# RS2002/PianoBart

Measured on AMD Instinct MI355X. Metric: Octuple tokens/sec/GPU (seq=1024, 12L/768d) pretrain step; %MFMA peak, higher is better.
Workload: dtype bf16

## Files before the change

### pianobart_amd/csrc/pb_fa_tiles.h

```cpp
#pragma once
#include "pb_common.h"
#include "pb_api_internal.h"

namespace {


constexpr int HD = 64, FT = 256;
constexpr float LOG2E = 1.4426950408889634f;
typedef __attribute__((ext_vector_type(4))) short s16x4;
typedef __attribute__((ext_vector_type(8))) short s16x8;

struct Fa64Args {
    const bf16_t *q, *k, *v, *o, *dout;
    bf16_t *out, *dq, *dk, *dv;
    float* lse; const float* delta; const float* key_mask; const int* kmax;
    int B, H, Sq, Sk;
    long q_sb, q_ss, k_sb, k_ss, v_sb, v_ss, o_sb, o_ss, dq_sb, dq_ss, dk_sb, dk_ss, dv_sb, dv_ss;
    float scale; int causal;
    float* cs_q; float* cs_kv;
    const bf16_t* zeros;
    const int *vl_q_off, *vl_k_off, *vl_q_len, *vl_k_len;
    const int* bh_order;
};

__device__ __forceinline__ void varlen_localize(Fa64Args& p, int b) {
    if (!p.vl_q_off) return;
    const long qo = p.vl_q_off[b], ko = p.vl_k_off[b];
    p.Sq = p.vl_q_len[b]; p.Sk = p.vl_k_len[b];
    p.q += qo * p.q_ss - b * p.q_sb; p.k += ko * p.k_ss - b * p.k_sb; p.v += ko * p.v_ss - b * p.v_sb;
    if (p.o) p.o += qo * p.o_ss - b * p.o_sb;
    if (p.out) p.out += qo * p.o_ss - b * p.o_sb;
    if (p.dout) p.dout += qo * p.o_ss - b * p.o_sb;
    if (p.dq) p.dq += qo * p.dq_ss - b * p.dq_sb;
    if (p.dk) p.dk += ko * p.dk_ss - b * p.dk_sb;
    if (p.dv) p.dv += ko * p.dv_ss - b * p.dv_sb;
}

#define MFMA16(a, b, c) __builtin_amdgcn_mfma_f32_16x16x32_bf16((a), (b), (c), 0, 0, 0)

__device__ __forceinline__ int fsw(int row) { return (((row >> 1) & 3) << 1) | ((row >> 3) & 1); }

__device__ __forceinline__ void glds16(const bf16_t* g, char* lds_wave_base) {
    __builtin_amdgcn_global_load_lds((const __attribute__((address_space(1))) void*)g,
                                     (__attribute__((address_space(3))) void*)lds_wave_base, 16, 0, 0);
}
struct StageOff { unsigned off[2]; unsigned chunk[2]; };
__device__ __forceinline__ StageOff stage_off(long ld, int wave, int lane) {
    StageOff o;
#pragma unroll
    for (int n = 0; n < 2; ++n) {
        const int row = (wave * 2 + n) * 8 + (lane >> 3);
        o.chunk[n] = (unsigned)((lane & 7) ^ fsw(row));
        o.off[n] = (unsigned)(row * ld + (o.chunk[n] << 3));
    }
    return o;
}
__device__ __forceinline__ void stage64(const bf16_t* __restrict__ base, long ld, int r0, int nrows, char* lds, int wave, int lane, const StageOff& so,
                                        int cmax = 8, const bf16_t* zeros = nullptr) {
    if (r0 + 64 <= nrows) {
        const bf16_t* tb = base + (long)r0 * ld;
#pragma unroll
        for (int n = 0; n < 2; ++n) glds16((cmax == 8 || (int)so.chunk[n] < cmax) ? tb + so.off[n] : zeros, lds + (wave * 2 + n) * 1024);
    } else {
#pragma unroll
        for (int n = 0; n < 2; ++n) {
            const int inst = wave * 2 + n;
            const int row = inst * 8 + (lane >> 3);
            const int chunk = (lane & 7) ^ fsw(row);
            const int gr = min(r0 + row, nrows - 1);
            glds16((cmax == 8 || chunk < cmax) ? base + (long)gr * ld + chunk * 8 : zeros, lds + inst * 1024);
        }
    }
}
__device__ __forceinline__ bf16x8 frag_row(const char* lds, int row, int ks, int g) {
    return *reinterpret_cast<const bf16x8*>(lds + row * 128 + (((ks * 4 + g) ^ fsw(row)) << 4));
}
__device__ __forceinline__ bf16x8 frag_tr(const char* lds, int c0, int s, int lane) {
    const int lr = lane & 15, g = lane >> 4, qq = lr >> 2, pp = lr & 3;
    const int chunk = (c0 >> 3) + (pp >> 1);
    const int r0 = 32 * s + 4 * g + qq, r1 = r0 + 16;
    const int o0 = r0 * 128 + ((chunk ^ fsw(r0)) << 4) + ((pp & 1) << 3);
    const int o1 = r1 * 128 + ((chunk ^ fsw(r1)) << 4) + ((pp & 1) << 3);
    const s16x4 lo = __builtin_amdgcn_ds_read_tr16_b64_v4i16((__attribute__((address_space(3))) s16x4*)(lds + o0));
    const s16x4 hi = __builtin_amdgcn_ds_read_tr16_b64_v4i16((__attribute__((address_space(3))) s16x4*)(lds + o1));
    const s16x8 v = {lo[0], lo[1], lo[2], lo[3], hi[0], hi[1], hi[2], hi[3]};
    return __builtin_bit_cast(bf16x8, v);
}
__device__ __forceinline__ bf16x8 pack_pair(const f32x4& lo, const f32x4& hi) {
    bf16x8 r = {(bf16_t)lo[0], (bf16_t)lo[1], (bf16_t)lo[2], (bf16_t)lo[3], (bf16_t)hi[0], (bf16_t)hi[1], (bf16_t)hi[2], (bf16_t)hi[3]};
    return r;
}
__device__ __forceinline__ bf16x8 frag_global(const bf16_t* __restrict__ g, long ld, int row, int nvalid, int col) {
    bf16x8 z = {};
    if (row < nvalid) z = *reinterpret_cast<const bf16x8*>(g + (long)row * ld + col);
    return z;
}
__device__ __forceinline__ float grp_max(float v) {
    auto a = __builtin_amdgcn_permlane16_swap(__float_as_uint(v), __float_as_uint(v), false, false);
    v = fmaxf(__uint_as_float(a[0]), __uint_as_float(a[1]));
    auto b = __builtin_amdgcn_permlane32_swap(__float_as_uint(v), __float_as_uint(v), false, false);
    return fmaxf(__uint_as_float(b[0]), __uint_as_float(b[1]));
}
__device__ __forceinline__ float grp_sum(float v) {
    auto a = __builtin_amdgcn_permlane16_swap(__float_as_uint(v), __float_as_uint(v), false, false);
    v = __uint_as_float(a[0]) + __uint_as_float(a[1]);
    auto b = __builtin_amdgcn_permlane32_swap(__float_as_uint(v), __float_as_uint(v), false, false);
    return __uint_as_float(b[0]) + __uint_as_float(b[1]);
}
template <bool V> struct BoolTag { static constexpr bool value = V; };

constexpr int STG = 2 * 8192 + 512;

__device__ __forceinline__ void block_map(int nrb, int H, int B, int& rb, int& h, int& b, const int* order = nullptr) {
    const int L = blockIdx.x, BH = H * B;
    int bh;
    if ((BH & 7) == 0) { const int x = L & 7, slot = L >> 3, j = slot / nrb; bh = j * 8 + x; rb = (slot - j * nrb + j) % nrb; }
    else { bh = L / nrb; rb = (L - bh * nrb + bh) % nrb; }
    if (order) bh = order[bh];
    h = bh % H; b = bh / H;
}

template <int OFF>
__device__ __forceinline__ void ds_tr(s16x4& d, unsigned addr) {
    asm volatile("ds_read_b64_tr_b16 %0, %1 offset:%2" : "=v"(d) : "v"(addr), "i"(OFF));
}
__device__ __forceinline__ unsigned tr_lane_off64(int c0, int lane) {
    const int lr = lane & 15, g = lane >> 4, qq = lr >> 2, pp = lr & 3;
    const int r0 = 4 * g + qq, chunk = (c0 >> 3) + (pp >> 1);
    return (unsigned)(r0 * 128 + ((chunk ^ fsw(r0)) << 4) + ((pp & 1) << 3));
}
__device__ __forceinline__ void ds_tr_block(s16x4 (&d)[2][2], unsigned addr) {
    ds_tr<0>(d[0][0], addr); ds_tr<2048>(d[0][1], addr); ds_tr<4096>(d[1][0], addr); ds_tr<6144>(d[1][1], addr);
}
__device__ __forceinline__ bf16x8 tr_join(s16x4 lo, s16x4 hi) {
    const s16x8 v = {lo[0], lo[1], lo[2], lo[3], hi[0], hi[1], hi[2], hi[3]};
    return __builtin_bit_cast(bf16x8, v);
}
#define TRW4(X) "+v"(X[0][0]), "+v"(X[0][1]), "+v"(X[1][0]), "+v"(X[1][1])
__device__ __forceinline__ void tr_wait4(s16x4 (&t)[4][2][2]) {
    asm volatile("s_waitcnt lgkmcnt(0)" : TRW4(t[0]), TRW4(t[1]), TRW4(t[2]), TRW4(t[3]));
}
__device__ __forceinline__ void tr_wait8(s16x4 (&t)[4][2][2], s16x4 (&u)[4][2][2]) {
    asm volatile("s_waitcnt lgkmcnt(0)" : TRW4(t[0]), TRW4(t[1]), TRW4(t[2]), TRW4(t[3]), TRW4(u[0]), TRW4(u[1]), TRW4(u[2]), TRW4(u[3]));
}
#undef TRW4
__device__ __forceinline__ unsigned lds_u32(const void* p) { return (unsigned)(uintptr_t)(__attribute__((address_space(3))) const char*)p; }

template <int N> __device__ __forceinline__ void wait_vm() { asm volatile("s_waitcnt vmcnt(%0)" :: "i"(N) : "memory"); }

template <int NB> struct FaCfg {
    static constexpr int NS = NB == 1 ? 3 : 2;
    static constexpr int STB = 2 * NB * 8192;
    static constexpr int PCS = 4 * NB;
    static constexpr int KT = NB == 1 ? 2 : 1;
};

__device__ __forceinline__ bf16x8 scale_frag(bf16x8 v, float c) {
    bf16x8 r;
#pragma unroll
    for (int e = 0; e < 8; ++e) r[e] = (bf16_t)((float)v[e] * c);
    return r;
}

}
```

### pianobart_amd/csrc/pb_flash64.hip

```cpp
#include "pb_common.h"
#include "pb_fa_tiles.h"

namespace {


constexpr float LAZY_THR = 8.0f;
template <int HD>
__global__ __launch_bounds__(FT) void fa64_fwd_kernel(const Fa64Args pin) {
    constexpr int NB = (HD + 63) / 64, KS = HD / 32, DT = HD / 16, HDT = HD;
    using C = FaCfg<NB>;
    extern __shared__ __attribute__((aligned(16))) char smem[];
    const int t = threadIdx.x, lane = t & 63, lr = lane & 15, g = lane >> 4;
    const int wave = __builtin_amdgcn_readfirstlane(t >> 6);
    int rb, h, b;
    block_map((pin.Sq + 127) / 128, pin.H, pin.B, rb, h, b, pin.bh_order);
    if (pin.causal) rb = (pin.Sq + 127) / 128 - 1 - rb;
    const int q0 = rb * 128;
    Fa64Args p = pin;
    varlen_localize(p, b);
    const int lse_ld = pin.Sq;
    if (q0 >= p.Sq) return;
    const bf16_t* Q = p.q + b * p.q_sb + h * HDT;
    const bf16_t* K = p.k + b * p.k_sb + h * HDT;
    const bf16_t* V = p.v + b * p.v_sb + h * HDT;
    const float c = p.scale * LOG2E;
    const int kvis_end = p.kmax ? min(p.Sk, p.kmax[b]) : p.Sk;
    const int kend = p.causal ? min(kvis_end, q0 + 128) : kvis_end;
    const int nt = (kend + 63) / 64;
    float* ldsBias = reinterpret_cast<float*>(smem + C::NS * C::STB);
    unsigned* ldsFlag = reinterpret_cast<unsigned*>(ldsBias + ((p.Sk + 63) / 64) * 64);
    for (int tile = wave; tile < nt; tile += 4) {
        const int key = tile * 64 + lane;
        const bool vis = key < (pin.vl_q_off ? kvis_end : p.Sk) && (!p.key_mask || p.key_mask[(long)b * p.Sk + key] != 0.f);
        ldsBias[key] = vis ? 0.f : -INFINITY;
        const bool allvis = __builtin_amdgcn_ballot_w64(vis) == ~0ull;
        if (lane == 0) ldsFlag[tile] = allvis ? 0u : 1u;
    }
    int myq[2];
    bf16x8 qf[2][KS];
#pragma unroll
    for (int qt = 0; qt < 2; ++qt) {
        myq[qt] = q0 + wave * 32 + qt * 16 + lr;
#pragma unroll
        for (int ks = 0; ks < KS; ++ks) qf[qt][ks] = scale_frag(frag_global(Q, p.q_ss, myq[qt], p.Sq, ks * 32 + g * 8), c);
    }
#pragma unroll
    for (int ks = 0; ks < KS; ++ks) asm volatile("" : "+v"(qf[0][ks]), "+v"(qf[1][ks]));
    f32x4 oacc[2][DT];
#pragma unroll
    for (int qt = 0; qt < 2; ++qt)
#pragma unroll
        for (int i = 0; i < DT; ++i) oacc[qt][i] = f32x4{0.f, 0.f, 0.f, 0.f};
    float m[2] = {-INFINITY, -INFINITY};
    f32x4 cinit[2] = {f32x4{0.f, 0.f, 0.f, 0.f}, f32x4{0.f, 0.f, 0.f, 0.f}};
    f32x4 lacc[2] = {f32x4{0.f, 0.f, 0.f, 0.f}, f32x4{0.f, 0.f, 0.f, 0.f}};
    const bf16_t one = (bf16_t)1.0f;
    const bf16x8 ones = {one, one, one, one, one, one, one, one};
    unsigned voff[4];
#pragma unroll
    for (int dt = 0; dt < 4; ++dt) voff[dt] = lds_u32(smem) + NB * 8192 + tr_lane_off64(dt * 16, lane);
    const StageOff so_k = stage_off(p.k_ss, wave, lane), so_v = stage_off(p.v_ss, wave, lane);
    auto stage = [&](int it, int sidx) {
        char* st = smem + sidx * C::STB;
#pragma unroll
        for (int nb = 0; nb < NB; ++nb) {
            stage64(K + nb * 64, p.k_ss, it * 64, p.Sk, st + nb * 8192, wave, lane, so_k, min(8, (HD - nb * 64) / 8), p.zeros);
            stage64(V + nb * 64, p.v_ss, it * 64, p.Sk, st + (NB + nb) * 8192, wave, lane, so_v, min(8, (HD - nb * 64) / 8), p.zeros);
        }
    };
    if (nt > 0) stage(0, 0);
    if (C::NS == 3 && nt > 1) { stage(1, 1); wait_vm<C::PCS>(); } else { wait_vm<0>(); }
    __builtin_amdgcn_s_waitcnt(0xc07f);
    __builtin_amdgcn_s_barrier();
    int sidx = 0;
    for (int it = 0; it < nt; ++it) {
        const char* st = smem + sidx * C::STB;
        const int nidx = sidx == 0 ? C::NS - 1 : sidx - 1;
        if (it + C::NS - 1 < nt) stage(it + C::NS - 1, nidx);
        const float* ldsB = ldsBias + it * 64;
        const int k0 = it * 64;
        const bool diag = p.causal && (k0 + 63 > q0 + wave * 32);
        const bool masked = diag || __builtin_amdgcn_readfirstlane(ldsFlag[it]) != 0u;
        f32x4 s[2][4];
#pragma unroll
        for (int kt = 0; kt < 4; ++kt) {
#pragma unroll
            for (int qt = 0; qt < 2; ++qt) s[qt][kt] = cinit[qt];
#pragma unroll
            for (int nb = 0; nb < NB; ++nb) {
#pragma unroll
                for (int k2 = 0; k2 < 2; ++k2)
                    if (2 * nb + k2 < KS) {
                        const bf16x8 kk = frag_row(st + nb * 8192, kt * 16 + lr, k2, g);
#pragma unroll
                        for (int qt = 0; qt < 2; ++qt) s[qt][kt] = MFMA16(kk, qf[qt][2 * nb + k2], s[qt][kt]);
                    }
            }
        }
        s16x4 tv[4][2][2];
#pragma unroll
        for (int dt = 0; dt < 4; ++dt) if (dt < DT) ds_tr_block(tv[dt], voff[dt] + (unsigned)(sidx * C::STB));
        bf16x8 pf[2][2];
        auto finish_row = [&](int qt) {
            pf[qt][0] = pack_pair(s[qt][0], s[qt][1]);
            pf[qt][1] = pack_pair(s[qt][2], s[qt][3]);
            lacc[qt] = MFMA16(ones, pf[qt][1], MFMA16(ones, pf[qt][0], lacc[qt]));
        };
        float resc[2] = {1.f, 1.f};
        auto exact_tile = [&](auto tag) {
            constexpr bool MASKED = decltype(tag)::value;
            asm volatile("; exact softmax path" ::: "memory");
#pragma unroll
            for (int qt = 0; qt < 2; ++qt) {
                const float mold = m[qt] == -INFINITY ? 0.f : m[qt];
                float mx = -INFINITY;
#pragma unroll
                for (int kt = 0; kt < 4; ++kt) {
                    f32x4 bias = {0.f, 0.f, 0.f, 0.f};
                    if constexpr (MASKED) bias = *reinterpret_cast<const f32x4*>(ldsB + kt * 16 + g * 4);
#pragma unroll
                    for (int r = 0; r < 4; ++r) {
                        float x = s[qt][kt][r] + mold;
                        if constexpr (MASKED) {
                            x += bias[r];
                            if (diag && (k0 + kt * 16 + g * 4 + r) > myq[qt]) x = -INFINITY;
                        }
                        s[qt][kt][r] = x;
                        mx = fmaxf(mx, x);
                    }
                }
                mx = grp_max(mx);
                const float mnew = fmaxf(m[qt], mx);
                const float muse = mnew == -INFINITY ? 0.f : mnew;
                const float alpha = __builtin_amdgcn_exp2f(m[qt] - muse);
#pragma unroll
                for (int kt = 0; kt < 4; ++kt)
#pragma unroll
                    for (int r = 0; r < 4; ++r) s[qt][kt][r] = __builtin_amdgcn_exp2f(s[qt][kt][r] - muse);
                lacc[qt] *= alpha;
                m[qt] = mnew;
                cinit[qt] = f32x4{-muse, -muse, -muse, -muse};
                resc[qt] = alpha;
                finish_row(qt);
            }
        };
        bool exact = masked;
        if (masked) {
            exact_tile(BoolTag<true>{});
        } else {
            float t0 = m[0] == -INFINITY ? INFINITY : -INFINITY, t1 = m[1] == -INFINITY ? INFINITY : -INFINITY;
#pragma unroll
            for (int kt = 0; kt < 4; ++kt)
#pragma unroll
                for (int r = 0; r < 4; ++r) { t0 = fmaxf(t0, s[0][kt][r]); t1 = fmaxf(t1, s[1][kt][r]); }
            if (__builtin_amdgcn_ballot_w64(fmaxf(t0, t1) > LAZY_THR) == 0ull) {
#pragma unroll
                for (int qt = 0; qt < 2; ++qt) {
#pragma unroll
                    for (int kt = 0; kt < 4; ++kt)
#pragma unroll
                        for (int r = 0; r < 4; ++r) s[qt][kt][r] = __builtin_amdgcn_exp2f(s[qt][kt][r]);
                    finish_row(qt);
                }
            } else {
                exact = true;
                exact_tile(BoolTag<false>{});
            }
        }
        if (exact) {
#pragma unroll
            for (int qt = 0; qt < 2; ++qt)
#pragma unroll
                for (int i = 0; i < DT; ++i) oacc[qt][i] *= resc[qt];
        }
#pragma unroll
        for (int nb = 0; nb < NB; ++nb) {
            if (nb > 0) {
#pragma unroll
                for (int dt = 0; dt < 4; ++dt) if (nb * 4 + dt < DT) ds_tr_block(tv[dt], voff[dt] + (unsigned)(sidx * C::STB + nb * 8192));
            }
            tr_wait4(tv);
#pragma unroll
            for (int dt = 0; dt < 4; ++dt) if (nb * 4 + dt < DT) {
                const bf16x8 v0 = tr_join(tv[dt][0][0], tv[dt][0][1]), v1 = tr_join(tv[dt][1][0], tv[dt][1][1]);
#pragma unroll
                for (int qt = 0; qt < 2; ++qt) oacc[qt][nb * 4 + dt] = MFMA16(v1, pf[qt][1], MFMA16(v0, pf[qt][0], oacc[qt][nb * 4 + dt]));
            }
        }
        if (C::NS == 3 && it + 2 < nt) { wait_vm<C::PCS>(); } else { wait_vm<0>(); }
        __builtin_amdgcn_s_barrier();
        sidx = sidx == C::NS - 1 ? 0 : sidx + 1;
    }
    if constexpr (HD == 64) {
        typedef __attribute__((ext_vector_type(2))) unsigned u32x2;
        typedef __attribute__((ext_vector_type(4))) unsigned u32x4;
        const unsigned obase = lds_u32(smem) + (unsigned)(wave * 4096);
#pragma unroll
        for (int qt = 0; qt < 2; ++qt) {
            const float lq = lacc[qt][0];
            const float inv = lq > 0.f ? 1.0f / lq : 0.f;
#pragma unroll
            for (int dt = 0; dt < DT; ++dt) {
                const bf16x4 r = {(bf16_t)(oacc[qt][dt][0] * inv), (bf16_t)(oacc[qt][dt][1] * inv), (bf16_t)(oacc[qt][dt][2] * inv), (bf16_t)(oacc[qt][dt][3] * inv)};
                *reinterpret_cast<__attribute__((address_space(3))) u32x2*>(obase + (unsigned)(qt * 2048 + lr * 128 + ((((dt * 2 + (g >> 1)) ^ (lr & 7)) << 4) | ((g & 1) << 3)))) =
                    __builtin_bit_cast(u32x2, r);
            }
            if (myq[qt] < p.Sq && g == 0) p.lse[((long)b * p.H + h) * lse_ld + myq[qt]] = lq > 0.f ? (m[qt] + log2f(lq)) / LOG2E : INFINITY;
        }
        const int orow = lane >> 3, ochunk = lane & 7;
#pragma unroll
        for (int qt = 0; qt < 2; ++qt)
#pragma unroll
            for (int hh = 0; hh < 2; ++hh) {
                const int r = hh * 8 + orow, q = q0 + wave * 32 + qt * 16 + r;
                const u32x4 v = *reinterpret_cast<const __attribute__((address_space(3))) u32x4*>(obase + (unsigned)(qt * 2048 + r * 128 + ((ochunk ^ (r & 7)) << 4)));
                if (q < p.Sq) *reinterpret_cast<u32x4*>(p.out + b * p.o_sb + (long)q * p.o_ss + h * HDT + ochunk * 8) = v;
            }
    } else {
#pragma unroll
    for (int qt = 0; qt < 2; ++qt) {
        if (myq[qt] < p.Sq) {
            const float lq = lacc[qt][0];
            const float inv = lq > 0.f ? 1.0f / lq : 0.f;
            bf16_t* O = p.out + b * p.o_sb + (long)myq[qt] * p.o_ss + h * HDT;
#pragma unroll
            for (int dt = 0; dt < DT; ++dt) {
                bf16x4 r = {(bf16_t)(oacc[qt][dt][0] * inv), (bf16_t)(oacc[qt][dt][1] * inv), (bf16_t)(oacc[qt][dt][2] * inv), (bf16_t)(oacc[qt][dt][3] * inv)};
                *reinterpret_cast<bf16x4*>(O + dt * 16 + g * 4) = r;
            }
            if (g == 0) p.lse[((long)b * p.H + h) * lse_ld + myq[qt]] = lq > 0.f ? (m[qt] + log2f(lq)) / LOG2E : INFINITY;
        }
    }
    }
}

template <int HD>
__global__ __launch_bounds__(FT) void fa64_bwd_dkv_kernel(const Fa64Args pin) {
    constexpr int NB = (HD + 63) / 64, KS = HD / 32, DT = HD / 16, HDT = HD;
    using C = FaCfg<NB>;
    constexpr int KT = C::KT, BK_ = 64 * KT;
    extern __shared__ __attribute__((aligned(16))) char smem[];
    const int t = threadIdx.x, lane = t & 63, lr = lane & 15, g = lane >> 4;
    const int wave = __builtin_amdgcn_readfirstlane(t >> 6);
    int rb, h, b;
    block_map((pin.Sk + BK_ - 1) / BK_, pin.H, pin.B, rb, h, b, pin.bh_order);
    const int k0 = rb * BK_;
    Fa64Args p = pin;
    varlen_localize(p, b);
    const int lse_ld = pin.Sq;
    if (k0 >= p.Sk) {
        if (p.cs_kv && t < 2 * HDT) {
            const int nkb0 = (pin.Sk + BK_ - 1) / BK_, dm = p.H * HDT;
            float* row = p.cs_kv + (long)(b * nkb0 + rb) * 2 * dm + h * HDT;
            row[t < HDT ? t : dm + t - HDT] = 0.f;
        }
        return;
    }
    const bf16_t* Q = p.q + b * p.q_sb + h * HDT;
    const bf16_t* K = p.k + b * p.k_sb + h * HDT;
    const bf16_t* V = p.v + b * p.v_sb + h * HDT;
    const bf16_t* DO = p.dout + b * p.o_sb + h * HDT;
    const float c = p.scale * LOG2E;
    const int it0 = p.causal ? k0 / 64 : 0;
    const int nt = (p.kmax && k0 >= p.kmax[b]) ? 0 : (p.Sq + 63) / 64;
    const int sqp = ((p.Sq + 63) / 64) * 64;
    float* ldsNL = reinterpret_cast<float*>(smem + C::NS * C::STB);
    float* ldsND = ldsNL + sqp;
    {
        const long li0 = ((long)b * p.H + h) * lse_ld;
        for (int qb = it0 * 64; qb < nt * 64; qb += 4 * FT) {
            float tl[4], td[4];
#pragma unroll
            for (int i = 0; i < 4; ++i) {
                const int q = qb + t + i * FT;
                tl[i] = q < p.Sq ? p.lse[li0 + q] : INFINITY;
                td[i] = q < p.Sq ? p.delta[li0 + q] : 0.f;
            }
#pragma unroll
            for (int i = 0; i < 4; ++i) {
                const int q = qb + t + i * FT;
                if (q < nt * 64) { ldsNL[q] = tl[i] == INFINITY ? -INFINITY : -tl[i] * LOG2E; ldsND[q] = -td[i]; }
            }
        }
    }
    int mykey[KT];
    bf16x8 kf[KT][KS], vf[KT][KS];
#pragma unroll
    for (int kt = 0; kt < KT; ++kt) {
        mykey[kt] = k0 + wave * (16 * KT) + kt * 16 + lr;
#pragma unroll
        for (int ks = 0; ks < KS; ++ks) {
            kf[kt][ks] = scale_frag(frag_global(K, p.k_ss, mykey[kt], p.Sk, ks * 32 + g * 8), c);
            vf[kt][ks] = frag_global(V, p.v_ss, mykey[kt], p.Sk, ks * 32 + g * 8);
        }
    }
#pragma unroll
    for (int kt = 0; kt < KT; ++kt)
#pragma unroll
        for (int ks = 0; ks < KS; ++ks) asm volatile("" : "+v"(kf[kt][ks]), "+v"(vf[kt][ks]));
    f32x4 dk[KT][DT], dv[KT][DT];
#pragma unroll
    for (int kt = 0; kt < KT; ++kt)
#pragma unroll
        for (int i = 0; i < DT; ++i) { dk[kt][i] = f32x4{0.f, 0.f, 0.f, 0.f}; dv[kt][i] = f32x4{0.f, 0.f, 0.f, 0.f}; }
    unsigned qoff[4], ooff[4];
#pragma unroll
    for (int dt = 0; dt < 4; ++dt) { qoff[dt] = lds_u32(smem) + tr_lane_off64(dt * 16, lane); ooff[dt] = qoff[dt] + NB * 8192; }
    const StageOff so_q = stage_off(p.q_ss, wave, lane), so_o = stage_off(p.o_ss, wave, lane);
    auto stage = [&](int it, int sidx) {
        char* st = smem + sidx * C::STB;
#pragma unroll
        for (int nb = 0; nb < NB; ++nb) {
            stage64(Q + nb * 64, p.q_ss, it * 64, p.Sq, st + nb * 8192, wave, lane, so_q, min(8, (HD - nb * 64) / 8), p.zeros);
            stage64(DO + nb * 64, p.o_ss, it * 64, p.Sq, st + (NB + nb) * 8192, wave, lane, so_o, min(8, (HD - nb * 64) / 8), p.zeros);
        }
    };
    if (it0 < nt) stage(it0, 0);
    if (C::NS == 3 && it0 + 1 < nt) { stage(it0 + 1, 1); wait_vm<C::PCS>(); } else { wait_vm<0>(); }
    __builtin_amdgcn_s_waitcnt(0xc07f);
    __builtin_amdgcn_s_barrier();
    int sidx = 0;
    for (int it = it0; it < nt; ++it) {
        const char* st = smem + sidx * C::STB;
        const int nidx = sidx == 0 ? C::NS - 1 : sidx - 1;
        if (it + C::NS - 1 < nt) stage(it + C::NS - 1, nidx);
        const int q0 = it * 64;
        const bool diag = p.causal && (k0 + wave * (16 * KT) + 16 * KT - 1 > q0);
        bf16x8 pf[KT][2], df[KT][2];
#pragma unroll
        for (int half = 0; half < 2; ++half) {
            f32x4 sv[KT][2], dp[KT][2];
#pragma unroll
            for (int qq = 0; qq < 2; ++qq) {
                const int qt = half * 2 + qq;
                const f32x4 nl = *reinterpret_cast<const f32x4*>(ldsNL + q0 + qt * 16 + g * 4);
                const f32x4 nd = *reinterpret_cast<const f32x4*>(ldsND + q0 + qt * 16 + g * 4);
#pragma unroll
                for (int kt = 0; kt < KT; ++kt) { sv[kt][qq] = nl; dp[kt][qq] = nd; }
#pragma unroll
                for (int nb = 0; nb < NB; ++nb) {
                    const char* ldsQ = st + nb * 8192; const char* ldsO = st + (NB + nb) * 8192;
#pragma unroll
                    for (int k2 = 0; k2 < 2; ++k2)
                        if (2 * nb + k2 < KS) {
                            const bf16x8 qa = frag_row(ldsQ, qt * 16 + lr, k2, g), oa = frag_row(ldsO, qt * 16 + lr, k2, g);
#pragma unroll
                            for (int kt = 0; kt < KT; ++kt) {
                                sv[kt][qq] = MFMA16(qa, kf[kt][2 * nb + k2], sv[kt][qq]);
                                dp[kt][qq] = MFMA16(oa, vf[kt][2 * nb + k2], dp[kt][qq]);
                            }
                        }
                }
            }
            if (diag) {
#pragma unroll
                for (int kt = 0; kt < KT; ++kt)
#pragma unroll
                    for (int qq = 0; qq < 2; ++qq)
#pragma unroll
                        for (int r = 0; r < 4; ++r) {
                            const int q = q0 + (half * 2 + qq) * 16 + g * 4 + r;
                            const float pr = mykey[kt] <= q ? __builtin_amdgcn_exp2f(sv[kt][qq][r]) : 0.f;
                            sv[kt][qq][r] = pr; dp[kt][qq][r] *= pr;
                        }
            } else {
#pragma unroll
                for (int kt = 0; kt < KT; ++kt)
#pragma unroll
                    for (int qq = 0; qq < 2; ++qq)
#pragma unroll
                        for (int r = 0; r < 4; ++r) {
                            const float pr = __builtin_amdgcn_exp2f(sv[kt][qq][r]);
                            sv[kt][qq][r] = pr; dp[kt][qq][r] *= pr;
                        }
            }
#pragma unroll
            for (int kt = 0; kt < KT; ++kt) { pf[kt][half] = pack_pair(sv[kt][0], sv[kt][1]); df[kt][half] = pack_pair(dp[kt][0], dp[kt][1]); }
        }
#pragma unroll
        for (int nb = 0; nb < NB; ++nb)
#pragma unroll
        for (int si = 0; si < 2; ++si) {
            s16x4 to[4][2], tq[4][2];
#pragma unroll
            for (int dt = 0; dt < 4; ++dt) if (nb * 4 + dt < DT) {
                const unsigned ao = ooff[dt] + (unsigned)(sidx * C::STB + nb * 8192), aq = qoff[dt] + (unsigned)(sidx * C::STB + nb * 8192);
                if (si == 0) { ds_tr<0>(to[dt][0], ao); ds_tr<2048>(to[dt][1], ao); ds_tr<0>(tq[dt][0], aq); ds_tr<2048>(tq[dt][1], aq); }
                else { ds_tr<4096>(to[dt][0], ao); ds_tr<6144>(to[dt][1], ao); ds_tr<4096>(tq[dt][0], aq); ds_tr<6144>(tq[dt][1], aq); }
            }
            asm volatile("s_waitcnt lgkmcnt(0)" : "+v"(to[0][0]), "+v"(to[0][1]), "+v"(to[1][0]), "+v"(to[1][1]), "+v"(to[2][0]), "+v"(to[2][1]), "+v"(to[3][0]), "+v"(to[3][1]),
                                                  "+v"(tq[0][0]), "+v"(tq[0][1]), "+v"(tq[1][0]), "+v"(tq[1][1]), "+v"(tq[2][0]), "+v"(tq[2][1]), "+v"(tq[3][0]), "+v"(tq[3][1]));
#pragma unroll
            for (int dt = 0; dt < 4; ++dt) if (nb * 4 + dt < DT) {
                const bf16x8 ot = tr_join(to[dt][0], to[dt][1]), qtf = tr_join(tq[dt][0], tq[dt][1]);
#pragma unroll
                for (int kt = 0; kt < KT; ++kt) {
                    dv[kt][nb * 4 + dt] = MFMA16(ot, pf[kt][si], dv[kt][nb * 4 + dt]);
                    dk[kt][nb * 4 + dt] = MFMA16(qtf, df[kt][si], dk[kt][nb * 4 + dt]);
                }
            }
        }
        if (C::NS == 3 && it + 2 < nt) { wait_vm<C::PCS>(); } else { wait_vm<0>(); }
        __builtin_amdgcn_s_barrier();
        sidx = sidx == C::NS - 1 ? 0 : sidx + 1;
    }
    f32x4 csk[DT], csv[DT];
#pragma unroll
    for (int dt = 0; dt < DT; ++dt) { csk[dt] = f32x4{0.f, 0.f, 0.f, 0.f}; csv[dt] = f32x4{0.f, 0.f, 0.f, 0.f}; }
    if constexpr (HD == 64) {
        typedef __attribute__((ext_vector_type(2))) unsigned u32x2;
        typedef __attribute__((ext_vector_type(4))) unsigned u32x4;
        const unsigned obase = lds_u32(smem) + 4096u + (unsigned)(wave * (KT * 4096));
#pragma unroll
        for (int kt = 0; kt < KT; ++kt) {
            const int key = k0 + wave * (16 * KT) + kt * 16 + lr;
            const bool kvis = pin.vl_q_off ? key < (p.kmax ? p.kmax[b] : p.Sk)
                                           : (!p.key_mask || p.key_mask[(long)b * p.Sk + (key < p.Sk ? key : 0)] != 0.f);
#pragma unroll
            for (int dt = 0; dt < DT; ++dt) {
                f32x4 vk = dk[kt][dt] * p.scale, vv = dv[kt][dt];
                if (!kvis) { vk = f32x4{0.f, 0.f, 0.f, 0.f}; vv = f32x4{0.f, 0.f, 0.f, 0.f}; }
                const bf16x4 rk = {(bf16_t)vk[0], (bf16_t)vk[1], (bf16_t)vk[2], (bf16_t)vk[3]}, rv = {(bf16_t)vv[0], (bf16_t)vv[1], (bf16_t)vv[2], (bf16_t)vv[3]};
                const unsigned slot = (unsigned)(lr * 128 + ((((dt * 2 + (g >> 1)) ^ (lr & 7)) << 4) | ((g & 1) << 3)));
                *reinterpret_cast<__attribute__((address_space(3))) u32x2*>(obase + (unsigned)(kt * 4096) + slot) = __builtin_bit_cast(u32x2, rk);
                *reinterpret_cast<__attribute__((address_space(3))) u32x2*>(obase + (unsigned)(kt * 4096 + 2048) + slot) = __builtin_bit_cast(u32x2, rv);
                if (key < p.Sk) { csk[dt] += vk; csv[dt] += vv; }
            }
        }
        const int orow = lane >> 3, ochunk = lane & 7;
#pragma unroll
        for (int kt = 0; kt < KT; ++kt)
#pragma unroll
            for (int hh = 0; hh < 2; ++hh) {
                const int r = hh * 8 + orow, key = k0 + wave * (16 * KT) + kt * 16 + r;
                const unsigned slot = (unsigned)(r * 128 + ((ochunk ^ (r & 7)) << 4));
                const u32x4 vk = *reinterpret_cast<const __attribute__((address_space(3))) u32x4*>(obase + (unsigned)(kt * 4096) + slot);
                const u32x4 vv = *reinterpret_cast<const __attribute__((address_space(3))) u32x4*>(obase + (unsigned)(kt * 4096 + 2048) + slot);
                if (key < p.Sk) {
                    *reinterpret_cast<u32x4*>(p.dk + b * p.dk_sb + (long)key * p.dk_ss + h * HDT + ochunk * 8) = vk;
                    *reinterpret_cast<u32x4*>(p.dv + b * p.dv_sb + (long)key * p.dv_ss + h * HDT + ochunk * 8) = vv;
                }
            }
    } else {
#pragma unroll
    for (int kt = 0; kt < KT; ++kt) {
        const int key = k0 + wave * (16 * KT) + kt * 16 + lr;
        const bool kvis = pin.vl_q_off ? key < (p.kmax ? p.kmax[b] : p.Sk)
                                       : (!p.key_mask || p.key_mask[(long)b * p.Sk + (key < p.Sk ? key : 0)] != 0.f);
        bf16_t* DK = p.dk + b * p.dk_sb + (long)key * p.dk_ss + h * HDT + g * 4;
        bf16_t* DV = p.dv + b * p.dv_sb + (long)key * p.dv_ss + h * HDT + g * 4;
#pragma unroll
        for (int dt = 0; dt < DT; ++dt) {
            f32x4 vk = dk[kt][dt] * p.scale, vv = dv[kt][dt];
            if (!kvis) { vk = f32x4{0.f, 0.f, 0.f, 0.f}; vv = f32x4{0.f, 0.f, 0.f, 0.f}; }
            if (key < p.Sk) {
                bf16x4 rk = {(bf16_t)vk[0], (bf16_t)vk[1], (bf16_t)vk[2], (bf16_t)vk[3]}, rv = {(bf16_t)vv[0], (bf16_t)vv[1], (bf16_t)vv[2], (bf16_t)vv[3]};
                *reinterpret_cast<bf16x4*>(DK + dt * 16) = rk;
                *reinterpret_cast<bf16x4*>(DV + dt * 16) = rv;
                csk[dt] += vk; csv[dt] += vv;
            }
        }
    }
    }
    if (p.cs_kv) {
        const int nkb = (pin.Sk + BK_ - 1) / BK_, d_model = p.H * HDT;
        float* red = reinterpret_cast<float*>(smem);
#pragma unroll
        for (int dt = 0; dt < DT; ++dt) {
#pragma unroll
            for (int e = 0; e < 4; ++e) {
                float v = csk[dt][e], u = csv[dt][e];
                v += PB_DPP_F(v, 0x140); u += PB_DPP_F(u, 0x140);
                v += PB_DPP_F(v, 0x141); u += PB_DPP_F(u, 0x141);
                v += PB_DPP_F(v, 0x4e); u += PB_DPP_F(u, 0x4e);
                v += PB_DPP_F(v, 0xb1); u += PB_DPP_F(u, 0xb1);
                csk[dt][e] = v; csv[dt][e] = u;
            }
            if (lr == 0) {
                *reinterpret_cast<f32x4*>(red + wave * 2 * HDT + dt * 16 + g * 4) = csk[dt];
                *reinterpret_cast<f32x4*>(red + wave * 2 * HDT + HDT + dt * 16 + g * 4) = csv[dt];
            }
        }
        __syncthreads();
        if (t < 2 * HDT) {
            float* row = p.cs_kv + (long)(b * nkb + rb) * 2 * d_model + h * HDT;
            const float v = red[t] + red[2 * HDT + t] + red[4 * HDT + t] + red[6 * HDT + t];
            row[t < HDT ? t : d_model + t - HDT] = v;
        }
    }
}

template <int HD>
__global__ __launch_bounds__(FT) void fa64_bwd_dq_kernel(const Fa64Args pin) {
    constexpr int NB = (HD + 63) / 64, KS = HD / 32, DT = HD / 16, HDT = HD;
    using C = FaCfg<NB>;
    extern __shared__ __attribute__((aligned(16))) char smem[];
    const int t = threadIdx.x, lane = t & 63, lr = lane & 15, g = lane >> 4;
    const int wave = __builtin_amdgcn_readfirstlane(t >> 6);
    int rb, h, b;
    block_map((pin.Sq + 127) / 128, pin.H, pin.B, rb, h, b, pin.bh_order);
    if (pin.causal) rb = (pin.Sq + 127) / 128 - 1 - rb;
    const int q0 = rb * 128;
    Fa64Args p = pin;
    varlen_localize(p, b);
    const int lse_ld = pin.Sq;
    if (q0 >= p.Sq) {
        if (p.cs_q && t < HDT) p.cs_q[(long)(b * ((pin.Sq + 127) / 128) + rb) * (p.H * HDT) + h * HDT + t] = 0.f;
        return;
    }
    const bf16_t* Q = p.q + b * p.q_sb + h * HDT;
    const bf16_t* K = p.k + b * p.k_sb + h * HDT;
    const bf16_t* V = p.v + b * p.v_sb + h * HDT;
    const bf16_t* DO = p.dout + b * p.o_sb + h * HDT;
    const float c = p.scale * LOG2E;
    const int kvis_end = p.kmax ? min(p.Sk, p.kmax[b]) : p.Sk;
    const int kend = p.causal ? min(kvis_end, q0 + 128) : kvis_end;
    const int nt = (kend + 63) / 64;
    float* ldsBias = reinterpret_cast<float*>(smem + C::NS * C::STB);
    unsigned* ldsFlag = reinterpret_cast<unsigned*>(ldsBias + ((p.Sk + 63) / 64) * 64);
    for (int tile = wave; tile < nt; tile += 4) {
        const int key = tile * 64 + lane;
        const bool vis = key < (pin.vl_q_off ? kvis_end : p.Sk) && (!p.key_mask || p.key_mask[(long)b * p.Sk + key] != 0.f);
        ldsBias[key] = vis ? 0.f : -INFINITY;
        const bool allvis = __builtin_amdgcn_ballot_w64(vis) == ~0ull;
        if (lane == 0) ldsFlag[tile] = allvis ? 0u : 1u;
    }
    int myq[2];
    bf16x8 qf[2][KS], of[2][KS];
    float nl[2], nd[2];
#pragma unroll
    for (int qt = 0; qt < 2; ++qt) {
        myq[qt] = q0 + wave * 32 + qt * 16 + lr;
        const long li = ((long)b * p.H + h) * lse_ld + myq[qt];
        const float ls = myq[qt] < p.Sq ? p.lse[li] : INFINITY;
        nl[qt] = ls == INFINITY ? -INFINITY : -ls * LOG2E;
        float dl = 0.f;
#pragma unroll
        for (int ks = 0; ks < KS; ++ks) {
            qf[qt][ks] = scale_frag(frag_global(Q, p.q_ss, myq[qt], p.Sq, ks * 32 + g * 8), c);
            of[qt][ks] = frag_global(DO, p.o_ss, myq[qt], p.Sq, ks * 32 + g * 8);
            const bf16x8 ov = frag_global(p.o + b * p.o_sb + h * HDT, p.o_ss, myq[qt], p.Sq, ks * 32 + g * 8);
#pragma unroll
            for (int e = 0; e < 8; ++e) dl = fmaf((float)of[qt][ks][e], (float)ov[e], dl);
        }
        dl = grp_sum(dl);
        nd[qt] = -dl;
        if (g == 0 && myq[qt] < p.Sq) const_cast<float*>(p.delta)[li] = dl;
    }
#pragma unroll
    for (int qt = 0; qt < 2; ++qt) {
#pragma unroll
        for (int ks = 0; ks < KS; ++ks) asm volatile("" : "+v"(qf[qt][ks]), "+v"(of[qt][ks]));
        asm volatile("" : "+v"(nl[qt]), "+v"(nd[qt]));
    }
    f32x4 dq[2][DT];
#pragma unroll
    for (int qt = 0; qt < 2; ++qt)
#pragma unroll
        for (int i = 0; i < DT; ++i) dq[qt][i] = f32x4{0.f, 0.f, 0.f, 0.f};
    unsigned koff[4];
#pragma unroll
    for (int dt = 0; dt < 4; ++dt) koff[dt] = lds_u32(smem) + tr_lane_off64(dt * 16, lane);
    const StageOff so_k = stage_off(p.k_ss, wave, lane), so_v = stage_off(p.v_ss, wave, lane);
    auto stage = [&](int it, int sidx) {
        char* st = smem + sidx * C::STB;
#pragma unroll
        for (int nb = 0; nb < NB; ++nb) {
            stage64(K + nb * 64, p.k_ss, it * 64, p.Sk, st + nb * 8192, wave, lane, so_k, min(8, (HD - nb * 64) / 8), p.zeros);
            stage64(V + nb * 64, p.v_ss, it * 64, p.Sk, st + (NB + nb) * 8192, wave, lane, so_v, min(8, (HD - nb * 64) / 8), p.zeros);
        }
    };
    if (nt > 0) stage(0, 0);
    if (C::NS == 3 && nt > 1) { stage(1, 1); wait_vm<C::PCS>(); } else { wait_vm<0>(); }
    __builtin_amdgcn_s_waitcnt(0xc07f);
    __builtin_amdgcn_s_barrier();
    int sidx = 0;
    for (int it = 0; it < nt; ++it) {
        const char* st = smem + sidx * C::STB;
        const int nidx = sidx == 0 ? C::NS - 1 : sidx - 1;
        if (it + C::NS - 1 < nt) stage(it + C::NS - 1, nidx);
        const float* ldsB = ldsBias + it * 64;
        const int k0 = it * 64;
        const bool diag = p.causal && (k0 + 63 > q0 + wave * 32);
        const bool masked = __builtin_amdgcn_readfirstlane(ldsFlag[it]) != 0u;
        bf16x8 df[2][2];
#pragma unroll
        for (int half = 0; half < 2; ++half) {
            f32x4 ds_[2][2];
#pragma unroll
            for (int kk = 0; kk < 2; ++kk) {
                const int kt = half * 2 + kk;
                f32x4 sv[2], dpv[2];
#pragma unroll
                for (int qt = 0; qt < 2; ++qt) { sv[qt] = f32x4{nl[qt], nl[qt], nl[qt], nl[qt]}; dpv[qt] = f32x4{nd[qt], nd[qt], nd[qt], nd[qt]}; }
#pragma unroll
                for (int nb = 0; nb < NB; ++nb) {
                    const char* ldsK = st + nb * 8192; const char* ldsV = st + (NB + nb) * 8192;
#pragma unroll
                    for (int k2 = 0; k2 < 2; ++k2)
                        if (2 * nb + k2 < KS) {
                            const bf16x8 ka = frag_row(ldsK, kt * 16 + lr, k2, g), va = frag_row(ldsV, kt * 16 + lr, k2, g);
#pragma unroll
                            for (int qt = 0; qt < 2; ++qt) {
                                sv[qt] = MFMA16(ka, qf[qt][2 * nb + k2], sv[qt]);
                                dpv[qt] = MFMA16(va, of[qt][2 * nb + k2], dpv[qt]);
                            }
                        }
                }
#pragma unroll
                for (int qt = 0; qt < 2; ++qt) {
                    if (masked) sv[qt] += *reinterpret_cast<const f32x4*>(ldsB + kt * 16 + g * 4);
                    if (diag) {
#pragma unroll
                        for (int r = 0; r < 4; ++r) if (k0 + kt * 16 + g * 4 + r > myq[qt]) sv[qt][r] = -INFINITY;
                    }
#pragma unroll
                    for (int r = 0; r < 4; ++r) dpv[qt][r] *= __builtin_amdgcn_exp2f(sv[qt][r]);
                    ds_[qt][kk] = dpv[qt];
                }
            }
#pragma unroll
            for (int qt = 0; qt < 2; ++qt) df[qt][half] = pack_pair(ds_[qt][0], ds_[qt][1]);
        }
#pragma unroll
        for (int nb = 0; nb < NB; ++nb) {
            s16x4 tk[4][2][2];
#pragma unroll
            for (int dt = 0; dt < 4; ++dt) if (nb * 4 + dt < DT) ds_tr_block(tk[dt], koff[dt] + (unsigned)(sidx * C::STB + nb * 8192));
            tr_wait4(tk);
#pragma unroll
            for (int dt = 0; dt < 4; ++dt) if (nb * 4 + dt < DT) {
                const bf16x8 k0f = tr_join(tk[dt][0][0], tk[dt][0][1]), k1f = tr_join(tk[dt][1][0], tk[dt][1][1]);
#pragma unroll
                for (int qt = 0; qt < 2; ++qt) dq[qt][nb * 4 + dt] = MFMA16(k1f, df[qt][1], MFMA16(k0f, df[qt][0], dq[qt][nb * 4 + dt]));
            }
        }
        if (C::NS == 3 && it + 2 < nt) { wait_vm<C::PCS>(); } else { wait_vm<0>(); }
        __builtin_amdgcn_s_barrier();
        sidx = sidx == C::NS - 1 ? 0 : sidx + 1;
    }
    f32x4 csq[DT];
#pragma unroll
    for (int dt = 0; dt < DT; ++dt) csq[dt] = f32x4{0.f, 0.f, 0.f, 0.f};
    if constexpr (HD == 64) {
        typedef __attribute__((ext_vector_type(2))) unsigned u32x2;
        typedef __attribute__((ext_vector_type(4))) unsigned u32x4;
        const unsigned obase = lds_u32(smem) + 4096u + (unsigned)(wave * 4096);
#pragma unroll
        for (int qt = 0; qt < 2; ++qt)
#pragma unroll
            for (int dt = 0; dt < DT; ++dt) {
                const f32x4 v = dq[qt][dt] * p.scale;
                const bf16x4 r = {(bf16_t)v[0], (bf16_t)v[1], (bf16_t)v[2], (bf16_t)v[3]};
                *reinterpret_cast<__attribute__((address_space(3))) u32x2*>(obase + (unsigned)(qt * 2048 + lr * 128 + ((((dt * 2 + (g >> 1)) ^ (lr & 7)) << 4) | ((g & 1) << 3)))) =
                    __builtin_bit_cast(u32x2, r);
                if (myq[qt] < p.Sq) csq[dt] += v;
            }
        const int orow = lane >> 3, ochunk = lane & 7;
#pragma unroll
        for (int qt = 0; qt < 2; ++qt)
#pragma unroll
            for (int hh = 0; hh < 2; ++hh) {
                const int r = hh * 8 + orow, q = q0 + wave * 32 + qt * 16 + r;
                const u32x4 v = *reinterpret_cast<const __attribute__((address_space(3))) u32x4*>(obase + (unsigned)(qt * 2048 + r * 128 + ((ochunk ^ (r & 7)) << 4)));
                if (q < p.Sq) *reinterpret_cast<u32x4*>(p.dq + b * p.dq_sb + (long)q * p.dq_ss + h * HDT + ochunk * 8) = v;
            }
    } else {
#pragma unroll
    for (int qt = 0; qt < 2; ++qt)
        if (myq[qt] < p.Sq) {
            bf16_t* DQ = p.dq + b * p.dq_sb + (long)myq[qt] * p.dq_ss + h * HDT;
#pragma unroll
            for (int dt = 0; dt < DT; ++dt) {
                const f32x4 v = dq[qt][dt] * p.scale;
                bf16x4 r = {(bf16_t)v[0], (bf16_t)v[1], (bf16_t)v[2], (bf16_t)v[3]};
                *reinterpret_cast<bf16x4*>(DQ + dt * 16 + g * 4) = r;
                csq[dt] += v;
            }
        }
    }
    if (p.cs_q) {
        const int nqb = (pin.Sq + 127) / 128, d_model = p.H * HDT;
        float* red = reinterpret_cast<float*>(smem);
#pragma unroll
        for (int dt = 0; dt < DT; ++dt) {
#pragma unroll
            for (int e = 0; e < 4; ++e) {
                float v = csq[dt][e];
                v += __builtin_bit_cast(float, __builtin_amdgcn_update_dpp(0, __builtin_bit_cast(int, v), 0x140, 0xf, 0xf, true));
                v += __builtin_bit_cast(float, __builtin_amdgcn_update_dpp(0, __builtin_bit_cast(int, v), 0x141, 0xf, 0xf, true));
                v += __builtin_bit_cast(float, __builtin_amdgcn_update_dpp(0, __builtin_bit_cast(int, v), 0x4e, 0xf, 0xf, true));
                v += __builtin_bit_cast(float, __builtin_amdgcn_update_dpp(0, __builtin_bit_cast(int, v), 0xb1, 0xf, 0xf, true));
                csq[dt][e] = v;
            }
            if (lr == 0) *reinterpret_cast<f32x4*>(red + wave * HDT + dt * 16 + g * 4) = csq[dt];
        }
        __syncthreads();
        if (t < HDT) p.cs_q[(long)(b * nqb + rb) * d_model + h * HDT + t] = red[t] + red[HDT + t] + red[2 * HDT + t] + red[3 * HDT + t];
    }
}

}

static const bf16_t* fa_zero_page() {
    static void* pages[64] = {};
    int dev = 0;
    if (hipGetDevice(&dev) != hipSuccess || dev < 0 || dev >= 64) return nullptr;
    if (!pages[dev]) {
        void* p = nullptr;
        if (hipMalloc(&p, 256) != hipSuccess || hipMemset(p, 0, 256) != hipSuccess) return nullptr;
        pages[dev] = p;
    }
    return (const bf16_t*)pages[dev];
}

template <int HD>
static int fa64_fwd_launch(const Fa64Args& a, hipStream_t stream) {
    using C = FaCfg<(HD + 63) / 64>;
    const size_t lds = (size_t)C::NS * C::STB + (size_t)((a.Sk + 63) / 64) * (64 * 4 + 4);
    PB_REQUIRE(lds <= 160 * 1024, "pb_flash_fwd: Sk=%d needs %zu bytes of LDS", a.Sk, lds);
    if (lds > 65536) hipFuncSetAttribute(reinterpret_cast<const void*>(fa64_fwd_kernel<HD>), hipFuncAttributeMaxDynamicSharedMemorySize, (int)lds);
    hipLaunchKernelGGL(fa64_fwd_kernel<HD>, dim3(((a.Sq + 127) / 128) * a.H * a.B), dim3(FT), lds, stream, a);
    PB_LAUNCH_CHECK();
    return 0;
}

int pb_flash64_fwd(const void* q, const void* k, const void* v, void* o, float* lse, const float* key_mask, const int* kmax, int B, int H, int Sq, int Sk, int hd,
                   long q_sb, long q_ss, long k_sb, long k_ss, long v_sb, long v_ss, long o_sb, long o_ss, float scale, int causal, hipStream_t stream,
                   const int* const* vl) {
    Fa64Args a = {};
    if (vl) { a.vl_q_off = vl[0]; a.vl_q_len = vl[1]; a.vl_k_off = vl[2]; a.vl_k_len = vl[3]; a.bh_order = vl[4]; }
    a.q = (const bf16_t*)q; a.k = (const bf16_t*)k; a.v = (const bf16_t*)v; a.out = (bf16_t*)o; a.lse = lse; a.key_mask = key_mask; a.kmax = kmax;
    a.B = B; a.H = H; a.Sq = Sq; a.Sk = Sk; a.q_sb = q_sb; a.q_ss = q_ss; a.k_sb = k_sb; a.k_ss = k_ss; a.v_sb = v_sb; a.v_ss = v_ss;
    a.o_sb = o_sb; a.o_ss = o_ss; a.scale = scale; a.causal = causal;
    a.zeros = fa_zero_page();
    PB_REQUIRE(a.zeros != nullptr, "pb_flash_fwd: cannot allocate the zero page");
    return hd == 128 ? fa64_fwd_launch<128>(a, stream) : hd == 96 ? fa64_fwd_launch<96>(a, stream) : fa64_fwd_launch<64>(a, stream);
}

template <int HD>
static int fa64_bwd_launch(const Fa64Args& a, hipStream_t stream) {
    using C = FaCfg<(HD + 63) / 64>;
    const size_t lds_dkv = (size_t)C::NS * C::STB + (size_t)((a.Sq + 63) / 64) * 64 * 8;
    const size_t lds_dq = (size_t)C::NS * C::STB + (size_t)((a.Sk + 63) / 64) * (64 * 4 + 4);
    PB_REQUIRE(lds_dkv <= 160 * 1024 && lds_dq <= 160 * 1024, "pb_flash_bwd: Sq=%d Sk=%d need %zu / %zu bytes of LDS", a.Sq, a.Sk, lds_dkv, lds_dq);
    if (lds_dkv > 65536) hipFuncSetAttribute(reinterpret_cast<const void*>(fa64_bwd_dkv_kernel<HD>), hipFuncAttributeMaxDynamicSharedMemorySize, (int)lds_dkv);
    if (lds_dq > 65536) hipFuncSetAttribute(reinterpret_cast<const void*>(fa64_bwd_dq_kernel<HD>), hipFuncAttributeMaxDynamicSharedMemorySize, (int)lds_dq);
    constexpr int BK_ = 64 * C::KT;
    hipLaunchKernelGGL(fa64_bwd_dq_kernel<HD>, dim3(((a.Sq + 127) / 128) * a.H * a.B), dim3(FT), lds_dq, stream, a);
    PB_LAUNCH_CHECK();
    hipLaunchKernelGGL(fa64_bwd_dkv_kernel<HD>, dim3(((a.Sk + BK_ - 1) / BK_) * a.H * a.B), dim3(FT), lds_dkv, stream, a);
    PB_LAUNCH_CHECK();
    return 0;
}

int pb_flash64_bwd(const void* q, const void* k, const void* v, const void* o, const void* dout, const float* lse, float* delta, const float* key_mask,
                   const int* kmax, void* dq, void* dk, void* dv, int B, int H, int Sq, int Sk, int hd, long q_sb, long q_ss, long k_sb, long k_ss, long v_sb,
                   long v_ss, long o_sb, long o_ss, long dq_sb, long dq_ss, long dk_sb, long dk_ss, long dv_sb, long dv_ss, float scale,
                   int causal, float* dbias_q, float* dbias_k, float* dbias_v, float* dbias_ws, hipStream_t stream, const int* const* vl) {
    Fa64Args a = {};
    if (vl) { a.vl_q_off = vl[0]; a.vl_q_len = vl[1]; a.vl_k_off = vl[2]; a.vl_k_len = vl[3]; a.bh_order = vl[4]; }
    a.q = (const bf16_t*)q; a.k = (const bf16_t*)k; a.v = (const bf16_t*)v; a.o = (const bf16_t*)o; a.dout = (const bf16_t*)dout;
    a.dq = (bf16_t*)dq; a.dk = (bf16_t*)dk; a.dv = (bf16_t*)dv; a.lse = const_cast<float*>(lse); a.delta = delta; a.key_mask = key_mask; a.kmax = kmax;
    a.B = B; a.H = H; a.Sq = Sq; a.Sk = Sk; a.q_sb = q_sb; a.q_ss = q_ss; a.k_sb = k_sb; a.k_ss = k_ss; a.v_sb = v_sb; a.v_ss = v_ss;
    a.o_sb = o_sb; a.o_ss = o_ss; a.dq_sb = dq_sb; a.dq_ss = dq_ss; a.dk_sb = dk_sb; a.dk_ss = dk_ss; a.dv_sb = dv_sb; a.dv_ss = dv_ss;
    a.scale = scale; a.causal = causal;
    a.zeros = fa_zero_page();
    PB_REQUIRE(a.zeros != nullptr, "pb_flash_bwd: cannot allocate the zero page");
    const int kt_ = hd == 64 ? 2 : 1, nkb = (Sk + 64 * kt_ - 1) / (64 * kt_), nqb = (Sq + 127) / 128, d_model = H * hd;
    if (dbias_q) {
        PB_REQUIRE(dbias_k && dbias_v && dbias_ws, "pb_flash_bwd: dbias_q/k/v and dbias_ws go together");
        const size_t n_kv = (size_t)B * nkb * 2 * d_model;
        if (float* slice = pb_defer_alloc(n_kv + (size_t)B * nqb * d_model)) dbias_ws = slice;
        a.cs_kv = dbias_ws; a.cs_q = dbias_ws + n_kv;
    }
    const int rc = hd == 128 ? fa64_bwd_launch<128>(a, stream) : hd == 96 ? fa64_bwd_launch<96>(a, stream) : fa64_bwd_launch<64>(a, stream);
    if (rc || !dbias_q) return rc;
    if (pb_finalize_rows(a.cs_kv, B * nkb, d_model, dbias_k, stream, 2, dbias_v)) return -1;
    return pb_finalize_rows(a.cs_q, B * nqb, d_model, dbias_q, stream);
}

extern "C" int64_t pb_flash_bias_ws_floats(int32_t B, int32_t H, int32_t Sq, int32_t Sk, int32_t hd) {
    const int kt_ = hd == 64 ? 2 : 1, nkb = (Sk + 64 * kt_ - 1) / (64 * kt_), nqb = (Sq + 63) / 64;
    return (int64_t)B * H * hd * (2 * nkb + nqb);
}
```

Baseline: 623,900.

## Unify lazy softmax path and scalarize K/V staging addresses in flash forward

Restructures the forward attention inner loop so the exp2/pack/row-sum tail is shared between the lazy and exact rescale paths. A wave-uniform `noref` flag replaces the per-element -inf checks when deciding whether the running max must be rebased, and the oacc rescale moves inside the exact branch. K/V staging now goes through a paired helper that uses readfirstlane-uniform base pointers and precomputed byte offsets, aiming to cut VALU address arithmetic and register pressure. Asm barriers pin the constants and offsets in registers, which may change scheduling and register allocation.

After: 627,900 (median of 6 runs). Within noise of the previous version (+0.6%).

```diff
diff --git a/pianobart_amd/csrc/pb_fa_tiles.h b/pianobart_amd/csrc/pb_fa_tiles.h
--- a/pianobart_amd/csrc/pb_fa_tiles.h
+++ b/pianobart_amd/csrc/pb_fa_tiles.h
@@ -72,6 +72,42 @@
         }
     }
 }
+__device__ __forceinline__ const char* uniform_ptr(const void* p) {
+    const unsigned long long u = (unsigned long long)(uintptr_t)p;
+    const unsigned lo = __builtin_amdgcn_readfirstlane((unsigned)u), hi = __builtin_amdgcn_readfirstlane((unsigned)(u >> 32));
+    return (const char*)(uintptr_t)(((unsigned long long)hi << 32) | lo);
+}
+struct StageByteOff { unsigned a[2], b[2]; };
+__device__ __forceinline__ StageByteOff stage_byte_off(const StageOff& so_a, const StageOff& so_b) {
+    return StageByteOff{{so_a.off[0] * 2u, so_a.off[1] * 2u}, {so_b.off[0] * 2u, so_b.off[1] * 2u}};
+}
+__device__ __forceinline__ void stage_byte_off_keep(StageByteOff& bo) { asm volatile("" : "+v"(bo.a[0]), "+v"(bo.a[1]), "+v"(bo.b[0]), "+v"(bo.b[1])); }
+template <int NB, int HDIM>
+__device__ __forceinline__ void stage64_pair(const bf16_t* __restrict__ A, long lda, const bf16_t* __restrict__ B, long ldb, int r0, int nrows, char* st,
+                                             int wave, int lane, const StageOff& so_a, const StageOff& so_b, const StageByteOff& bo, const bf16_t* zeros) {
+    if (r0 + 64 <= nrows) {
+#pragma unroll
+        for (int nb = 0; nb < NB; ++nb) {
+            const int cmax = (HDIM - nb * 64) / 8 < 8 ? (HDIM - nb * 64) / 8 : 8;
+            const char* ta = uniform_ptr(A + nb * 64 + (long)r0 * lda);
+            const char* tb = uniform_ptr(B + nb * 64 + (long)r0 * ldb);
+            const unsigned* oa = bo.a; const unsigned* ob = bo.b;
+#pragma unroll
+            for (int n = 0; n < 2; ++n)
+                glds16((cmax == 8 || (int)so_a.chunk[n] < cmax) ? reinterpret_cast<const bf16_t*>(ta + oa[n]) : zeros, st + nb * 8192 + (wave * 2 + n) * 1024);
+#pragma unroll
+            for (int n = 0; n < 2; ++n)
+                glds16((cmax == 8 || (int)so_b.chunk[n] < cmax) ? reinterpret_cast<const bf16_t*>(tb + ob[n]) : zeros, st + (NB + nb) * 8192 + (wave * 2 + n) * 1024);
+        }
+    } else {
+#pragma unroll
+        for (int nb = 0; nb < NB; ++nb) {
+            const int cmax = (HDIM - nb * 64) / 8 < 8 ? (HDIM - nb * 64) / 8 : 8;
+            stage64(A + nb * 64, lda, r0, nrows, st + nb * 8192, wave, lane, so_a, cmax, zeros);
+            stage64(B + nb * 64, ldb, r0, nrows, st + (NB + nb) * 8192, wave, lane, so_b, cmax, zeros);
+        }
+    }
+}
 __device__ __forceinline__ bf16x8 frag_row(const char* lds, int row, int ks, int g) {
     return *reinterpret_cast<const bf16x8*>(lds + row * 128 + (((ks * 4 + g) ^ fsw(row)) << 4));
 }
diff --git a/pianobart_amd/csrc/pb_flash64.hip b/pianobart_amd/csrc/pb_flash64.hip
--- a/pianobart_amd/csrc/pb_flash64.hip
+++ b/pianobart_amd/csrc/pb_flash64.hip
@@ -55,18 +55,16 @@
     f32x4 cinit[2] = {f32x4{0.f, 0.f, 0.f, 0.f}, f32x4{0.f, 0.f, 0.f, 0.f}};
     f32x4 lacc[2] = {f32x4{0.f, 0.f, 0.f, 0.f}, f32x4{0.f, 0.f, 0.f, 0.f}};
     const bf16_t one = (bf16_t)1.0f;
-    const bf16x8 ones = {one, one, one, one, one, one, one, one};
+    bf16x8 ones = {one, one, one, one, one, one, one, one};
+    asm volatile("" : "+v"(ones));
+    bool noref = true;
     unsigned voff[4];
 #pragma unroll
     for (int dt = 0; dt < 4; ++dt) voff[dt] = lds_u32(smem) + NB * 8192 + tr_lane_off64(dt * 16, lane);
     const StageOff so_k = stage_off(p.k_ss, wave, lane), so_v = stage_off(p.v_ss, wave, lane);
+    StageByteOff so_b = stage_byte_off(so_k, so_v);
     auto stage = [&](int it, int sidx) {
-        char* st = smem + sidx * C::STB;
-#pragma unroll
-        for (int nb = 0; nb < NB; ++nb) {
-            stage64(K + nb * 64, p.k_ss, it * 64, p.Sk, st + nb * 8192, wave, lane, so_k, min(8, (HD - nb * 64) / 8), p.zeros);
-            stage64(V + nb * 64, p.v_ss, it * 64, p.Sk, st + (NB + nb) * 8192, wave, lane, so_v, min(8, (HD - nb * 64) / 8), p.zeros);
-        }
+        stage64_pair<NB, HD>(K, p.k_ss, V, p.v_ss, it * 64, p.Sk, smem + sidx * C::STB, wave, lane, so_k, so_v, so_b, p.zeros);
     };
     if (nt > 0) stage(0, 0);
     if (C::NS == 3 && nt > 1) { stage(1, 1); wait_vm<C::PCS>(); } else { wait_vm<0>(); }
@@ -76,7 +74,9 @@
     for (int it = 0; it < nt; ++it) {
         const char* st = smem + sidx * C::STB;
         const int nidx = sidx == 0 ? C::NS - 1 : sidx - 1;
+        stage_byte_off_keep(so_b);
         if (it + C::NS - 1 < nt) stage(it + C::NS - 1, nidx);
+        asm volatile("" : "+v"(lacc[0]), "+v"(lacc[1]));
         const float* ldsB = ldsBias + it * 64;
         const int k0 = it * 64;
         const bool diag = p.causal && (k0 + 63 > q0 + wave * 32);
@@ -100,78 +100,71 @@
         s16x4 tv[4][2][2];
 #pragma unroll
         for (int dt = 0; dt < 4; ++dt) if (dt < DT) ds_tr_block(tv[dt], voff[dt] + (unsigned)(sidx * C::STB));
-        bf16x8 pf[2][2];
-        auto finish_row = [&](int qt) {
-            pf[qt][0] = pack_pair(s[qt][0], s[qt][1]);
-            pf[qt][1] = pack_pair(s[qt][2], s[qt][3]);
-            lacc[qt] = MFMA16(ones, pf[qt][1], MFMA16(ones, pf[qt][0], lacc[qt]));
-        };
-        float resc[2] = {1.f, 1.f};
-        auto exact_tile = [&](auto tag) {
-            constexpr bool MASKED = decltype(tag)::value;
+        bool exact = masked || noref;
+        if (!exact) {
+            float tmax = s[0][0][0];
+#pragma unroll
+            for (int kt = 0; kt < 4; ++kt)
+#pragma unroll
+                for (int r = 0; r < 4; ++r) {
+                    if (kt + r > 0) tmax = fmaxf(tmax, s[0][kt][r]);
+                    tmax = fmaxf(tmax, s[1][kt][r]);
+                }
+            exact = __builtin_amdgcn_ballot_w64(tmax > LAZY_THR) != 0ull;
+        }
+        if (exact) {
             asm volatile("; exact softmax path" ::: "memory");
 #pragma unroll
             for (int qt = 0; qt < 2; ++qt) {
                 const float mold = m[qt] == -INFINITY ? 0.f : m[qt];
+#pragma unroll
+                for (int kt = 0; kt < 4; ++kt) s[qt][kt] += mold;
+            }
+            if (masked) {
+#pragma unroll
+                for (int kt = 0; kt < 4; ++kt) {
+                    const f32x4 bias = *reinterpret_cast<const f32x4*>(ldsB + kt * 16 + g * 4);
+#pragma unroll
+                    for (int qt = 0; qt < 2; ++qt)
+#pragma unroll
+                        for (int r = 0; r < 4; ++r) {
+                            float x = s[qt][kt][r] + bias[r];
+                            if (diag && (k0 + kt * 16 + g * 4 + r) > myq[qt]) x = -INFINITY;
+                            s[qt][kt][r] = x;
+                        }
+                }
+            }
+#pragma unroll
+            for (int qt = 0; qt < 2; ++qt) {
                 float mx = -INFINITY;
 #pragma unroll
-                for (int kt = 0; kt < 4; ++kt) {
-                    f32x4 bias = {0.f, 0.f, 0.f, 0.f};
-                    if constexpr (MASKED) bias = *reinterpret_cast<const f32x4*>(ldsB + kt * 16 + g * 4);
-#pragma unroll
-                    for (int r = 0; r < 4; ++r) {
-                        float x = s[qt][kt][r] + mold;
-                        if constexpr (MASKED) {
-                            x += bias[r];
-                            if (diag && (k0 + kt * 16 + g * 4 + r) > myq[qt]) x = -INFINITY;
-                        }
-                        s[qt][kt][r] = x;
-                        mx = fmaxf(mx, x);
-                    }
-                }
+                for (int kt = 0; kt < 4; ++kt)
+#pragma unroll
+                    for (int r = 0; r < 4; ++r) mx = fmaxf(mx, s[qt][kt][r]);
                 mx = grp_max(mx);
                 const float mnew = fmaxf(m[qt], mx);
                 const float muse = mnew == -INFINITY ? 0.f : mnew;
                 const float alpha = __builtin_amdgcn_exp2f(m[qt] - muse);
 #pragma unroll
-                for (int kt = 0; kt < 4; ++kt)
-#pragma unroll
-                    for (int r = 0; r < 4; ++r) s[qt][kt][r] = __builtin_amdgcn_exp2f(s[qt][kt][r] - muse);
+                for (int kt = 0; kt < 4; ++kt) s[qt][kt] -= muse;
                 lacc[qt] *= alpha;
+#pragma unroll
+                for (int i = 0; i < DT; ++i) oacc[qt][i] *= alpha;
                 m[qt] = mnew;
                 cinit[qt] = f32x4{-muse, -muse, -muse, -muse};
-                resc[qt] = alpha;
-                finish_row(qt);
-            }
-        };
-        bool exact = masked;
-        if (masked) {
-            exact_tile(BoolTag<true>{});
-        } else {
-            float t0 = m[0] == -INFINITY ? INFINITY : -INFINITY, t1 = m[1] == -INFINITY ? INFINITY : -INFINITY;
+            }
+            noref = __builtin_amdgcn_ballot_w64(m[0] == -INFINITY || m[1] == -INFINITY) != 0ull;
+        }
+        bf16x8 pf[2][2];
+#pragma unroll
+        for (int qt = 0; qt < 2; ++qt) {
 #pragma unroll
             for (int kt = 0; kt < 4; ++kt)
 #pragma unroll
-                for (int r = 0; r < 4; ++r) { t0 = fmaxf(t0, s[0][kt][r]); t1 = fmaxf(t1, s[1][kt][r]); }
-            if (__builtin_amdgcn_ballot_w64(fmaxf(t0, t1) > LAZY_THR) == 0ull) {
-#pragma unroll
-                for (int qt = 0; qt < 2; ++qt) {
-#pragma unroll
-                    for (int kt = 0; kt < 4; ++kt)
-#pragma unroll
-                        for (int r = 0; r < 4; ++r) s[qt][kt][r] = __builtin_amdgcn_exp2f(s[qt][kt][r]);
-                    finish_row(qt);
-                }
-            } else {
-                exact = true;
-                exact_tile(BoolTag<false>{});
-            }
-        }
-        if (exact) {
-#pragma unroll
-            for (int qt = 0; qt < 2; ++qt)
-#pragma unroll
-                for (int i = 0; i < DT; ++i) oacc[qt][i] *= resc[qt];
+                for (int r = 0; r < 4; ++r) s[qt][kt][r] = __builtin_amdgcn_exp2f(s[qt][kt][r]);
+            pf[qt][0] = pack_pair(s[qt][0], s[qt][1]);
+            pf[qt][1] = pack_pair(s[qt][2], s[qt][3]);
+            lacc[qt] = MFMA16(ones, pf[qt][1], MFMA16(ones, pf[qt][0], lacc[qt]));
         }
 #pragma unroll
         for (int nb = 0; nb < NB; ++nb) {
```
